# ramanathanlab/distllm

Hardware: NVIDIA B200
Metric: embedded chunks/sec @512-tok (higher is better)
Workload: dtype bf16

## Files before the change

### distllm_b200/_native.py

```python

from __future__ import annotations

import ctypes as C
from pathlib import Path

import torch

LIB_PATH = Path(__file__).resolve().parent / 'libb2e.so'
LIB_PATHS = {'f16': LIB_PATH, 'bf16': LIB_PATH.with_name('libb2e_bf16.so')}
STORAGE_TORCH_DTYPE = {'f16': torch.float16, 'bf16': torch.bfloat16}
_STORAGE_BY_ARCH = {'bert': 'bf16', 'esm': 'bf16', 'modernbert': 'bf16', 'mistral': 'f16'}


def storage_for_arch(arch: str) -> str:
    import os

    forced = os.environ.get('B2E_STORAGE')
    if forced:
        if forced not in LIB_PATHS:
            raise NativeError(f'B2E_STORAGE={forced!r}: expected one of {sorted(LIB_PATHS)}')
        return forced
    return _STORAGE_BY_ARCH[arch]


# ... 33 lines not shown
    'b2e_topk_ip',
    'b2e_topk_ip_tc',
    'b2e_max_row_norm',
    'b2e_pack_ubinary',
    'b2e_search_ubinary',
    'b2e_layernorm',
)
DEBUG_EXPORTS = (
    'b2e_debug_set_att3_clock',
    'b2e_debug_set_att3_flags',
    'b2e_debug_set_pair_flags',
    'b2e_debug_set_clock_buffer',
    'b2e_debug_set_layers',
    'b2e_debug_set_att3_variant',
    'b2e_debug_set_packing',
    'b2e_debug_topk_tc_fell_back',
    'b2e_debug_pack_layout',
    'b2e_debug_gemm_rows',
    'b2e_debug_attention_packed',
)


class NativeError(RuntimeError):
    """Raised when libb2e.so is missing or a native call fails."""


class ModelDesc(C.Structure):

    _fields_ = [
        ('arch', C.c_int32),
        ('num_layers', C.c_int32),
        ('hidden', C.c_int32),
        ('heads', C.c_int32),
# ... 249 lines not shown
                    epilogue: int, m_dev: torch.Tensor, out: torch.Tensor) -> torch.Tensor:
    lib = load(storage_of(a.dtype))
    for t, what in ((a, 'a'), (w, 'w'), (out, 'out'), (m_dev, 'm_dev')):
        _cuda_contig(t, what)
    if m_dev.dtype != torch.int32:
        raise NativeError('m_dev must be int32')
    m, k = a.shape
    n = w.shape[0]
    lib.b2e_debug_gemm_rows.argtypes = [C.c_void_p] * 5 + [C.c_int] * 4 + [C.c_void_p] * 2
    with torch.cuda.device(a.device):
        check(lib.b2e_debug_gemm_rows(a.data_ptr(), w.data_ptr(), _ptr(bias), _ptr(resid), out.data_ptr(), m, n, k,
                                      epilogue, m_dev.data_ptr(), stream_ptr(a.device)), lib)
    return out


def debug_attention_packed(qkv: torch.Tensor, attention_mask: torch.Tensor, cu: torch.Tensor, seq_len: torch.Tensor,
                           ctx: torch.Tensor, heads: int, kv_heads: int, head_dim: int, window: int = 0) -> torch.Tensor:
    lib = load(storage_of(qkv.dtype))
    for t, what in ((qkv, 'qkv'), (attention_mask, 'attention_mask'), (cu, 'cu'), (seq_len, 'len'), (ctx, 'ctx')):
        _cuda_contig(t, what)
    b, s = attention_mask.shape
    lib.b2e_debug_attention_packed.argtypes = [C.c_void_p] * 5 + [C.c_int] * 6 + [C.c_void_p]
    with torch.cuda.device(qkv.device):
        check(lib.b2e_debug_attention_packed(qkv.data_ptr(), attention_mask.data_ptr(), cu.data_ptr(),
                                             seq_len.data_ptr(), ctx.data_ptr(), b, s, heads, kv_heads, head_dim,
                                             window, stream_ptr(qkv.device)), lib)
    return ctx


def pack_ubinary(embeddings: torch.Tensor) -> torch.Tensor:
# ... 105 lines not shown
```

### distllm_b200/csrc/b2e_api.cu

```cuda
#include "../../include/b2e.h"
#include "../../include/b2e_debug.h"

#include <cuda.h>
#include <cuda_runtime.h>

#include <cstdarg>
#include <cstdio>
#include <cstdlib>
#include <cstring>
#include <string>
#include <utility>
#include <vector>

#include "attention3.cuh"
#include "attention4.cuh"
#include "attention5.cuh"
#include "binsearch.cuh"
#include "common.cuh"
#include "gemm.cuh"
#include "gemm2.cuh"
#include "mistral_ops.cuh"
#include "pack.cuh"
#include "rowops.cuh"
#include "topk.cuh"
// ... 217 lines not shown
bool g_gemm2_profiling = false;

template <int STAGES, int EPI>
int launch_gemm2_cfg(const CUtensorMap& ta, const CUtensorMap& tb, const CUtensorMap& tout,
                     const float* bias, const h16* resid, int M, int N, int K, int sms,
                     cudaStream_t st, const int* m_dev = nullptr) {
  using Cfg = Gemm2Cfg<STAGES>;
  const int tiles = ((M + 255) / 256) * (N / G2_BN);
  int grid = 2 * tiles;
  if (grid > (sms & ~1)) grid = sms & ~1;
  if constexpr (EPI == EPI_BIAS) {
    if (g_gemm2_profiling) {
      auto kern_tl = gemm2_h16_pair_kernel<STAGES, EPI, true>;
      const int arc = ensure_smem_attr(kern_tl, Cfg::SMEM_BYTES);
      if (arc) return arc;
      kern_tl<<<grid, G2_THREADS, Cfg::SMEM_BYTES, st>>>(ta, tb, tout, bias, resid, M, N, K, m_dev);
      CUDA_TRY(cudaGetLastError());
      return B2E_OK;
    }
  }
  auto kern = gemm2_h16_pair_kernel<STAGES, EPI>;
  {
    const int arc = ensure_smem_attr(kern, Cfg::SMEM_BYTES);
    if (arc) return arc;
  }
  kern<<<grid, G2_THREADS, Cfg::SMEM_BYTES, st>>>(ta, tb, tout, bias, resid, M, N, K, m_dev);
  CUDA_TRY(cudaGetLastError());
  return B2E_OK;
}

int launch_gemm(const CUtensorMap& ta, const CUtensorMap& tb, void* out, const float* bias,
                const void* resid, int M, int N, int K, int epi, int sms, cudaStream_t st,
                const int* m_dev = nullptr) {
  const h16* r = static_cast<const h16*>(resid);
  CUtensorMap tout;
  int rc;
  const bool glu = epi == B2E_EPI_SWIGLU || epi == B2E_EPI_GEGLU;
  const int n_out = glu ? N / 2 : N;
  if ((rc = make_tmap_h16(&tout, out, M, n_out, GEMM_OUT_BOX_ROWS))) return rc;
  if (N % 256 == 0 && gemm_use_pair()) {
    constexpr int PS = 5;
    switch (epi) {
      case B2E_EPI_BIAS: return launch_gemm2_cfg<PS, EPI_BIAS>(ta, tb, tout, bias, r, M, N, K, sms, st, m_dev);
      case B2E_EPI_BIAS_GELU: return launch_gemm2_cfg<PS, EPI_BIAS_GELU>(ta, tb, tout, bias, r, M, N, K, sms, st, m_dev);
      case B2E_EPI_BIAS_RESID: return launch_gemm2_cfg<PS, EPI_BIAS_RESID>(ta, tb, tout, bias, r, M, N, K, sms, st, m_dev);
      case B2E_EPI_SWIGLU: return launch_gemm2_cfg<PS, EPI_SWIGLU>(ta, tb, tout, bias, r, M, N, K, sms, st, m_dev);
      case B2E_EPI_GEGLU: return launch_gemm2_cfg<PS, EPI_GEGLU>(ta, tb, tout, bias, r, M, N, K, sms, st, m_dev);
    }
    return fail(B2E_ERR_INVALID, "unknown epilogue %d", epi);
  }
  if (N % 256 == 0) return launch_gemm_bn<256, 4>(ta, tb, tout, bias, r, M, N, K, epi, sms, st, m_dev);
  return launch_gemm_bn<128, 6>(ta, tb, tout, bias, r, M, N, K, epi, sms, st, m_dev);
}

struct AttnScratch {
  float* bias = nullptr;
  int* kv_chunks = nullptr;
  int* plain_chunks = nullptr;
  size_t cap_bias = 0, cap_b = 0;
  uint64_t gen = 0;
  int device = -1;
  int ensure(int B, int S_pad) {
    int dev = 0;
    CUDA_TRY(cudaGetDevice(&dev));
    if (dev != device) {
      release();
      device = dev;
// ... 389 lines not shown
    CUDA_TRY(cudaMalloc(&e->pk_src, sizeof(int) * tokens));
    e->pk_cap_t = tokens;
  }
  return e->pool.ensure(B, S, (size_t)B * pool_nsplit(S) * e->desc.hidden);
}

int g_packing = -1;
inline bool packing_enabled() {
  if (g_packing < 0) {
    const char* e = getenv("B2E_PACKED");
    g_packing = (e && e[0] == '0') ? 0 : 1;
  }
  return g_packing == 1;
}

int pack_prepare(B2EEncoder* e, const int64_t* mask, int B, int S, bool enable, cudaStream_t st, SeqLayout* lay) {
  pack_lengths_kernel<<<(B + 7) / 8, 256, 0, st>>>(mask, e->pk_len_raw, e->pk_ok, B, S);
  pack_scan_kernel<<<1, 256, 0, st>>>(e->pk_len_raw, e->pk_ok, e->pk_len, e->pk_cu, e->pk_treal, B, S,
                                      enable ? 1 : 0);
  pack_fill_kernel<<<dim3((S + 255) / 256, B), 256, 0, st>>>(e->pk_len, e->pk_cu, e->pk_src, B, S);
  CUDA_TRY(cudaGetLastError());
  lay->cu = e->pk_cu;
  lay->len = e->pk_len;
  lay->t_real = e->pk_treal;
  lay->tok_src = e->pk_src;
  return B2E_OK;
}

int validate_batch(const B2EEncoder* e, int B, int S) {
  if (!e) return fail(B2E_ERR_INVALID, "null encoder handle");
// ... 12 lines not shown
  const B2EModelDesc& d = e->desc;
  const int M = B * S, H = d.hidden, I = d.intermediate;
  int rc;
  DISPATCH_NV(H, (embed_layernorm_kernel<NV><<<row_blocks(M), ROW_THREADS, 0, st>>>(
                     ids, types, e->word(), e->pos(), e->type(), e->emb_g(), e->emb_b(), e->hidden,
                     M, S, d.eps, lay.t_real, lay.tok_src)));
  CUDA_TRY(cudaGetLastError());

  if ((rc = attention_prepare(e->attn, mask, B, S, st))) return rc;
  CUtensorMap tm_hidden, tm_ctx, tm_ffn, tm_qkv, tm_kv64;
  if ((rc = make_tmap_h16(&tm_kv64, e->qkv, M, 3 * H, AT3_KC))) return rc;
  if ((rc = make_tmap_h16(&tm_hidden, e->hidden, M, H, 128))) return rc;
  if ((rc = make_tmap_h16(&tm_ctx, e->ctx, M, H, 128))) return rc;
  if ((rc = make_tmap_h16(&tm_ffn, e->ffn, M, I, 128))) return rc;
  if ((rc = make_tmap_h16(&tm_qkv, e->qkv, M, 3 * H, 128))) return rc;

  for (int l = 0; l < d.num_layers; ++l) {
    if ((rc = launch_gemm(tm_hidden, e->tm_wqkv[l], e->qkv, (const float*)e->L(l, 1), nullptr, M,
                          3 * H, H, B2E_EPI_BIAS, e->sms, st, lay.t_real)))
      return rc;
    if ((rc = launch_attention(tm_qkv, tm_kv64, e->attn, e->ctx, B, S, d.heads, e->sms, st, 0, lay)))
      return rc;
    if ((rc = launch_gemm(tm_ctx, e->tm_wo[l], e->tmp, (const float*)e->L(l, 3), nullptr, M, H, H,
                          B2E_EPI_BIAS, e->sms, st, lay.t_real)))
      return rc;
    DISPATCH_NV(H, (layernorm_kernel<NV, h16><<<row_blocks(M), ROW_THREADS, 0, st>>>(
                       e->tmp, e->hidden, (const float*)e->L(l, 4), (const float*)e->L(l, 5),
                       e->hidden, M, d.eps, lay.t_real)));
    if ((rc = launch_gemm(tm_hidden, e->tm_w1[l], e->ffn, (const float*)e->L(l, 7), nullptr, M, I,
                          H, B2E_EPI_BIAS_GELU, e->sms, st, lay.t_real)))
      return rc;
    if ((rc = launch_gemm(tm_ffn, e->tm_w2[l], e->tmp, (const float*)e->L(l, 9), nullptr, M, H, I,
                          B2E_EPI_BIAS, e->sms, st, lay.t_real)))
      return rc;
    if (l + 1 < d.num_layers) {
      DISPATCH_NV(H, (layernorm_kernel<NV, h16><<<row_blocks(M), ROW_THREADS, 0, st>>>(
                         e->tmp, e->hidden, (const float*)e->L(l, 10), (const float*)e->L(l, 11),
                         e->hidden, M, d.eps, lay.t_real)));
    }
  }
  CUDA_TRY(cudaGetLastError());
  return B2E_OK;
}

int run_esm_trunk(B2EEncoder* e, const int64_t* ids, const int64_t* mask, int B, int S,
                  cudaStream_t st, const SeqLayout& lay = SeqLayout()) {
  const B2EModelDesc& d = e->desc;
  const int M = B * S, H = d.hidden, I = d.intermediate, L = d.num_layers;
  const int mask_token = d.reserved - 1;
  int rc;
  esm_token_scale_kernel<<<(B + 7) / 8, 256, 0, st>>>(ids, mask, e->tok_scale, B, S, mask_token);
  DISPATCH_NV(H, (esm_embed_kernel<NV><<<row_blocks(M), ROW_THREADS, 0, st>>>(
                     ids, mask, (const float*)e->w[0], e->tok_scale, e->xres, M, S, mask_token, lay.t_real,
// ... 145 lines not shown
int b2e_storage_dtype(void) { return kStorageDtype; }

int b2e_debug_set_att3_clock(void* device_buffer) {
  long long* p = static_cast<long long*>(device_buffer);
  CUDA_TRY(cudaMemcpyToSymbol(g_att3_clock, &p, sizeof(p)));
  return B2E_OK;
}

int b2e_debug_set_att3_flags(int flags) {
  CUDA_TRY(cudaMemcpyToSymbol(g_att3_flags, &flags, sizeof(flags)));
  return B2E_OK;
}

int b2e_debug_set_packing(int on) {
  g_packing = on ? 1 : 0;
  return B2E_OK;
}

int b2e_debug_set_att3_variant(int variant) {
  g_att3_variant = variant;
  return B2E_OK;
}

int b2e_debug_set_pair_flags(int flags) {
  g_gemm2_profiling = flags != 0;
  CUDA_TRY(cudaMemcpyToSymbol(g_gemm2_flags, &flags, sizeof(flags)));
  return B2E_OK;
}

int b2e_debug_set_clock_buffer(void* device_buffer) {
// ... 563 lines not shown
  if ((rc = make_tmap_h16(&tb, W, N, K, gemm_bn_for(N)))) return rc;
  return launch_gemm(ta, tb, out, bias, resid, M, N, K, epi, info.sms, (cudaStream_t)stream, m_dev);
}

int b2e_gemm_h16(const void* A, const void* W, const float* bias, const void* resid, void* out,
                  int M, int N, int K, int epi, void* stream) {
  return gemm_h16_checked(A, W, bias, resid, out, M, N, K, epi, nullptr, stream);
}

int b2e_debug_gemm_rows(const void* A, const void* W, const float* bias, const void* resid, void* out,
                        int M, int N, int K, int epi, const int* m_dev, void* stream) {
  if (!m_dev) return fail(B2E_ERR_INVALID, "gemm_rows: null device row count");
  return gemm_h16_checked(A, W, bias, resid, out, M, N, K, epi, m_dev, stream);
}

int b2e_attention_d64(const void* qkv, const int64_t* mask, void* ctx, int B, int S, int heads,
                      float* dbg, void* stream) {
  if (!qkv || !mask || !ctx) return fail(B2E_ERR_INVALID, "null tensor pointer");
  if (B <= 0 || S <= 0 || heads <= 0) return fail(B2E_ERR_INVALID, "empty attention problem");
  if (dbg) return fail(B2E_ERR_UNSUPPORTED, "the score dump of the first attention kernel is gone: pass NULL");
  int rc;
  DeviceInfo info;
  if ((rc = current_device_info(&info))) return rc;
  cudaStream_t st = (cudaStream_t)stream;
  CUtensorMap tq, tkv;
  if ((rc = make_tmap_h16(&tq, qkv, (uint64_t)B * S, (uint64_t)3 * heads * AT3_D, 128))) return rc;
  if ((rc = make_tmap_h16(&tkv, qkv, (uint64_t)B * S, (uint64_t)3 * heads * AT3_D, AT3_KC))) return rc;
  if ((rc = attention_prepare(g_attn_scratch, mask, B, S, st))) return rc;
  return launch_attention(tq, tkv, g_attn_scratch, ctx, B, S, heads, info.sms, st);
}
// ... 417 lines not shown
```

### distllm_b200/csrc/common.cuh

```cuda
#pragma once

#include <cuda.h>
#include <cuda_bf16.h>
#include <cuda_fp16.h>
#include <cuda_runtime.h>
#include <stdint.h>

namespace b2e {

using bf16 = __nv_bfloat16;
#ifdef B2E_STORAGE_BF16
using h16 = __nv_bfloat16;
#else
using h16 = __half;
#endif

__device__ __forceinline__ uint32_t smem_u32(const void* p) {
  return static_cast<uint32_t>(__cvta_generic_to_shared(p));
}

__device__ __forceinline__ uint32_t lane_id() { return threadIdx.x & 31u; }

__device__ __forceinline__ bool elect_one() {
  uint32_t pred = 0;
// ... 223 lines not shown
}
__device__ __forceinline__ void mbar_wait_cluster(uint32_t bar, uint32_t parity) {
  uint32_t ok = 0;
  while (!ok) {
    asm volatile(
        "{\n\t"
        ".reg .pred p;\n\t"
        "mbarrier.try_wait.parity.acquire.cluster.shared::cta.b64 p, [%1], %2;\n\t"
        "selp.u32 %0, 1, 0, p;\n\t"
        "}\n"
        : "=r"(ok)
        : "r"(bar), "r"(parity)
        : "memory");
  }
}
__device__ __forceinline__ void tma_load_2d_pair(uint32_t dst, const CUtensorMap* m,
                                                 uint32_t bar_cluster_addr, int c0, int c1) {
  asm volatile(
      "cp.async.bulk.tensor.2d.cta_group::2.shared::cluster.global.mbarrier::complete_tx::bytes"
      " [%0], [%1, {%3, %4}], [%2];"
      ::"r"(dst), "l"(m), "r"(bar_cluster_addr), "r"(c0), "r"(c1)
      : "memory");
}
__device__ __forceinline__ void tmem_alloc_pair(uint32_t smem_dst, uint32_t ncols) {
  asm volatile("tcgen05.alloc.cta_group::2.sync.aligned.shared::cta.b32 [%0], %1;" ::"r"(smem_dst),
               "r"(ncols)
               : "memory");
  asm volatile("tcgen05.relinquish_alloc_permit.cta_group::2.sync.aligned;" ::: "memory");
}
__device__ __forceinline__ void tmem_dealloc_pair(uint32_t taddr, uint32_t ncols) {
// ... 125 lines not shown
```

### distllm_b200/csrc/gemm.cuh

```cuda
#pragma once

#include "common.cuh"

namespace b2e {

enum GemmEpi : int { EPI_BIAS = 0, EPI_BIAS_GELU = 1, EPI_BIAS_RESID = 2, EPI_SWIGLU = 3, EPI_GEGLU = 4 };
__host__ __device__ constexpr bool epi_is_glu(int epi) { return epi == EPI_SWIGLU || epi == EPI_GEGLU; }

constexpr int GEMM_BM = 128;
constexpr int GEMM_BK = 64;
constexpr int GEMM_THREADS = 384;
constexpr int GEMM_EPI_WARPS = 8;
constexpr int GEMM_OUT_BOX_ROWS = 32;
constexpr int GEMM_STAGING_BYTES = GEMM_OUT_BOX_ROWS * 128;

template <int BN, int STAGES>
struct GemmCfg {
  static constexpr int A_BYTES = GEMM_BM * GEMM_BK * 2;
  static constexpr int B_BYTES = BN * GEMM_BK * 2;
  static constexpr int STAGE_BYTES = A_BYTES + B_BYTES;
  static constexpr int STAGING_OFFSET = STAGES * STAGE_BYTES;
  static constexpr int BAR_OFFSET = STAGING_OFFSET + GEMM_EPI_WARPS * GEMM_STAGING_BYTES;
  static constexpr int BIAS_OFFSET = BAR_OFFSET + 256;
  static constexpr int SMEM_BYTES = BIAS_OFFSET + 2 * BN * 4;
// ... 326 lines not shown
```

### distllm_b200/csrc/gemm2.cuh

```cuda
#pragma once

#include "common.cuh"
#include "gemm.cuh"

namespace b2e {

constexpr int G2_BN = 256;
constexpr int G2_THREADS = 384;
constexpr int G2_EPI_WARPS = 8;

template <int STAGES>
struct Gemm2Cfg {
  static constexpr int A_BYTES = 128 * GEMM_BK * 2;
  static constexpr int B_BYTES = (G2_BN / 2) * GEMM_BK * 2;
  static constexpr int STAGE_BYTES = A_BYTES + B_BYTES;
  static constexpr int STAGING_OFFSET = STAGES * STAGE_BYTES;
  static constexpr int STAGING_PER_WARP = 2 * GEMM_STAGING_BYTES;
  static constexpr int BAR_OFFSET = STAGING_OFFSET + G2_EPI_WARPS * STAGING_PER_WARP;
  static constexpr int SMEM_BYTES = BAR_OFFSET + 256;
  static constexpr int TMEM_COLS = 2 * G2_BN;
  static_assert(SMEM_BYTES <= 232448, "exceeds the 227 KiB per-CTA shared memory limit");
};

__device__ long long* g_gemm2_clock = nullptr;
__device__ int g_gemm2_flags = 0;

template <int STAGES, int EPI, bool TL = false>
__global__ void __cluster_dims__(2, 1, 1) __launch_bounds__(G2_THREADS, 1)
gemm2_h16_pair_kernel(const __grid_constant__ CUtensorMap tm_a,
                       const __grid_constant__ CUtensorMap tm_b,
                       const __grid_constant__ CUtensorMap tm_out,
                       const float* __restrict__ bias, const h16* __restrict__ resid, int M, int N,
                       int K, const int* __restrict__ m_dev) {
  if (m_dev != nullptr) M = __ldg(m_dev);
  using Cfg = Gemm2Cfg<STAGES>;
  extern __shared__ __align__(1024) uint8_t smem[];
  const uint32_t smem_base = smem_u32(smem);
  if ((smem_base & 1023u) != 0) __trap();

  const uint32_t full_bar = smem_base + Cfg::BAR_OFFSET;
  const uint32_t empty_bar = full_bar + 8u * STAGES;
  const uint32_t tfull_bar = empty_bar + 8u * STAGES;
  const uint32_t tempty_bar = tfull_bar + 16u;
  volatile uint32_t* tmem_slot =
      reinterpret_cast<volatile uint32_t*>(smem + Cfg::BAR_OFFSET + 8 * (2 * STAGES + 4));

  const int warp = threadIdx.x >> 5;
  const int lane = threadIdx.x & 31;
  const int flags = TL ? g_gemm2_flags : 0;
  const uint32_t rank = cluster_ctarank();
  const bool leader = rank == 0;

  if (warp == 0 && elect_one()) {
    tma_prefetch_desc(&tm_a);
    tma_prefetch_desc(&tm_b);
    tma_prefetch_desc(&tm_out);
  }
  if (warp == 1 && elect_one()) {
    for (int s = 0; s < STAGES; ++s) {
      mbar_init(full_bar + 8u * s, 1);
      mbar_init(empty_bar + 8u * s, 1);
    }
    for (int s = 0; s < 2; ++s) {
      mbar_init(tfull_bar + 8u * s, 1);
      mbar_init(tempty_bar + 8u * s, 2 * G2_EPI_WARPS);
    }
    mbar_fence_init();
  }
  cluster_sync_all();
  if (warp == 2) tmem_alloc_pair(smem_u32(const_cast<uint32_t*>(tmem_slot)), Cfg::TMEM_COLS);
  tc_fence_before();
  __syncthreads();
  tc_fence_after();
  const uint32_t tmem_base = *tmem_slot;

  const int m_pairs = (M + 255) / 256;
  const int n_tiles = N / G2_BN;
  const int total = m_pairs * n_tiles;
  const int kblocks = K / GEMM_BK;
  const int cluster_id = blockIdx.x >> 1;
  const int n_clusters = gridDim.x >> 1;
  long long* const clk = (TL && blockIdx.x < 2) ? g_gemm2_clock : nullptr;
  int clk_n = 0;
#define G2_STAMP(role)                                                                       \
  do {                                                                                       \
    if constexpr (TL) {                                                                      \
      if (clk != nullptr && clk_n < 256) clk[(blockIdx.x * 2 + (role)) * 256 + clk_n++] = clock64(); \
    }                                                                                        \
  } while (0)

  if (warp == 0) {
    if (elect_one()) {
      const uint32_t lead_full0 = mapa_shared(full_bar, 0);
      int stage = 0;
      uint32_t phase = 0;
      for (int tile = cluster_id; tile < total; tile += n_clusters) {
        const int m_pair = tile / n_tiles, n_blk = tile % n_tiles;
        const int row_a = m_pair * 256 + static_cast<int>(rank) * 128;
        const int row_b = n_blk * G2_BN + static_cast<int>(rank) * (G2_BN / 2);
        for (int kb = 0; kb < kblocks; ++kb) {
          mbar_wait(empty_bar + 8u * stage, phase ^ 1u);
          G2_STAMP(0);
          const uint32_t a_dst = smem_base + stage * Cfg::STAGE_BYTES;
          if (flags & 4) {
            if (leader) mbar_arrive(full_bar + 8u * stage);
          } else {
            if (leader) mbar_expect_tx(full_bar + 8u * stage, 2 * Cfg::STAGE_BYTES);
            const uint32_t fb = lead_full0 + 8u * stage;
            tma_load_2d_pair(a_dst, &tm_a, fb, kb * GEMM_BK, row_a);
            tma_load_2d_pair(a_dst + Cfg::A_BYTES, &tm_b, fb, kb * GEMM_BK, row_b);
          }
          if (++stage == STAGES) { stage = 0; phase ^= 1u; }
        }
      }
    }
  } else if (warp == 1) {
    if (leader && elect_one()) {
      constexpr uint32_t idesc = make_idesc_h16(256, G2_BN, 0, 0);
      int stage = 0;
      uint32_t phase = 0;
      int local = 0;
      for (int tile = cluster_id; tile < total; tile += n_clusters, ++local) {
        const int as = local & 1;
        const uint32_t aphase = (local >> 1) & 1u;
        mbar_wait_cluster(tempty_bar + 8u * as, aphase ^ 1u);
        tc_fence_after();
        const uint32_t d_tmem = tmem_base + static_cast<uint32_t>(as * G2_BN);
        for (int kb = 0; kb < kblocks; ++kb) {
          G2_STAMP(1);
          mbar_wait(full_bar + 8u * stage, phase);
          G2_STAMP(1);
          tc_fence_after();
          const uint32_t a_addr = smem_base + stage * Cfg::STAGE_BYTES;
          const uint64_t a_desc = make_smem_desc_sw128(a_addr, 16, 1024);
          const uint64_t b_desc = make_smem_desc_sw128(a_addr + Cfg::A_BYTES, 16, 1024);
          if (!(flags & 2)) {
#pragma unroll
            for (int k = 0; k < GEMM_BK / 16; ++k)
              tc_mma_f16_ss_pair(d_tmem, a_desc + 2u * k, b_desc + 2u * k, idesc,
                                 static_cast<uint32_t>((kb | k) != 0));
          }
          tc_commit_pair(empty_bar + 8u * stage, 3);
          G2_STAMP(1);
          if (++stage == STAGES) { stage = 0; phase ^= 1u; }
        }
        tc_commit_pair(tfull_bar + 8u * as, 3);
      }
    }
  } else if (warp >= 4) {
    const int q = warp & 3;
    const int half = (warp - 4) >> 2;
    constexpr int COLS_PER_WARP = G2_BN / 2;
    uint8_t* staging = smem + Cfg::STAGING_OFFSET + (warp - 4) * Cfg::STAGING_PER_WARP;
    const uint32_t staging_addr = smem_base + Cfg::STAGING_OFFSET + (warp - 4) * Cfg::STAGING_PER_WARP;
    const uint32_t lead_tempty0 = mapa_shared(tempty_bar, 0);
    const bool stamp = (warp == 4 && lane == 0 && !leader);
    int local = 0;
    for (int tile = cluster_id; tile < total; tile += n_clusters, ++local) {
      const int m_pair = tile / n_tiles, n_blk = tile % n_tiles;
      const int as = local & 1;
      const uint32_t aphase = (local >> 1) & 1u;
      const int row0 = m_pair * 256 + static_cast<int>(rank) * 128 + q * 32;
      const int row = row0 + lane;
      const bool row_ok = row < M;
      const int col0 = half * COLS_PER_WARP;
      const int gcol0 = n_blk * G2_BN + col0;
      const h16* resid_row =
          (EPI == EPI_BIAS_RESID) ? resid + static_cast<size_t>(row) * N + gcol0 : nullptr;

      if (stamp) G2_STAMP(1);
      if (flags & 16) {
        while (!mbar_test(tfull_bar + 8u * as, aphase)) __nanosleep(256);
      } else {
        mbar_wait(tfull_bar + 8u * as, aphase);
      }
      if (stamp) G2_STAMP(1);
      tc_fence_after();
      const uint32_t t_base = tmem_base + (static_cast<uint32_t>(q * 32) << 16) +
                              static_cast<uint32_t>(as * G2_BN + col0);
      if constexpr (epi_is_glu(EPI)) {
        uint32_t g[2][32], u[2][32];
        tmem_ld32(t_base, g[0]);
        tmem_ld32(t_base + 32u, g[1]);
        tmem_ld32(t_base + 64u, u[0]);
        tmem_ld32(t_base + 96u, u[1]);
        if (lane == 0) tma_store_wait_read<1>();
        __syncwarp();
        tmem_ld_wait();
        if (!(flags & 1)) {
          const int sidx = local & 1;
          gemm_swiglu_chunk<EPI == EPI_GEGLU>(g, u, staging + sidx * GEMM_STAGING_BYTES, lane);
          fence_proxy_async_smem();
          __syncwarp();
          if (lane == 0 && row0 < M) {
// ... 45 lines not shown
```

### include/b2e_debug.h

```cpp
#ifndef B2E_DEBUG_H_
#define B2E_DEBUG_H_

#include <stdint.h>

#ifdef __cplusplus
extern "C" {
#endif

struct B2EEncoder;
int b2e_debug_set_layers(struct B2EEncoder* enc, int n_layers);

int b2e_debug_set_att3_clock(void* device_buffer);
int b2e_debug_set_att3_flags(int flags);
int b2e_debug_set_packing(int on);
int b2e_debug_topk_tc_fell_back(int* out);
int b2e_debug_set_att3_variant(int variant);
int b2e_debug_set_pair_flags(int flags);
int b2e_debug_set_clock_buffer(void* device_buffer);

int b2e_debug_pack_layout(const int64_t* mask, int B, int S, int enable, int* cu, int* len, int* t_real,
                          int* tok_src, void* stream);
int b2e_debug_gemm_rows(const void* A, const void* W, const float* bias, const void* resid, void* out, int M,
                        int N, int K, int epi, const int* m_dev, void* stream);
int b2e_debug_attention_packed(const void* qkv, const int64_t* mask, const int* cu, const int* len, void* ctx,
                               int B, int S, int heads, int kv_heads, int head_dim, int window, void* stream);

#ifdef __cplusplus
}
#endif
#endif
```

Measured before the change: 9767.

## Fuse residual add and LayerNorm into the CTA-pair GEMM epilogue via cluster row-stat exchange

Adds a LayerNorm epilogue to the 2-CTA tcgen05 GEMM for BERT's attention-output and FFN-down projections. Clusters of 2*NP CTAs now cover the full hidden row (N<=1024). Each CTA TMA-loads the residual tile, computes partial mean and variance from TMEM, and exchanges them across the cluster with st.async. This removes the separate layernorm kernel launches and the round trip of the tmp buffer through global memory. In exchange, large clusters cap how many run at once and the grid is limited to M/256 clusters, which may underuse the SMs.

```diff
diff --git a/distllm_b200/_native.py b/distllm_b200/_native.py
--- a/distllm_b200/_native.py
+++ b/distllm_b200/_native.py
@@ -71,9 +71,12 @@
     'b2e_debug_set_layers',
     'b2e_debug_set_att3_variant',
     'b2e_debug_set_packing',
+    'b2e_debug_set_ln_fusion',
     'b2e_debug_topk_tc_fell_back',
     'b2e_debug_pack_layout',
     'b2e_debug_gemm_rows',
+    'b2e_debug_gemm_ln',
+    'b2e_debug_gemm_ln_max_clusters',
     'b2e_debug_attention_packed',
 )
 
@@ -353,6 +356,40 @@
     return out
 
 
+def debug_set_ln_fusion(on: bool, storage: str = 'bf16') -> None:
+    lib = load(storage)
+    lib.b2e_debug_set_ln_fusion.argtypes = [C.c_int]
+    check(lib.b2e_debug_set_ln_fusion(int(bool(on))), lib)
+
+
+def debug_gemm_ln(a: torch.Tensor, w: torch.Tensor, bias: torch.Tensor | None, resid: torch.Tensor,
+                  gamma: torch.Tensor, beta: torch.Tensor, eps: float, out: torch.Tensor,
+                  m_dev: torch.Tensor | None = None) -> torch.Tensor:
+    lib = load(storage_of(a.dtype))
+    for t, what in ((a, 'a'), (w, 'w'), (resid, 'resid'), (gamma, 'gamma'), (beta, 'beta'), (out, 'out')):
+        _cuda_contig(t, what)
+    if gamma.dtype != torch.float32 or beta.dtype != torch.float32:
+        raise NativeError('gamma and beta must be float32')
+    if m_dev is not None and m_dev.dtype != torch.int32:
+        raise NativeError('m_dev must be int32')
+    m, k = a.shape
+    n = w.shape[0]
+    lib.b2e_debug_gemm_ln.argtypes = [C.c_void_p] * 6 + [C.c_float, C.c_void_p] + [C.c_int] * 3 + [C.c_void_p] * 2
+    with torch.cuda.device(a.device):
+        check(lib.b2e_debug_gemm_ln(a.data_ptr(), w.data_ptr(), _ptr(bias), resid.data_ptr(), gamma.data_ptr(),
+                                    beta.data_ptr(), float(eps), out.data_ptr(), m, n, k, _ptr(m_dev),
+                                    stream_ptr(a.device)), lib)
+    return out
+
+
+def debug_gemm_ln_max_clusters(n: int, storage: str = 'bf16') -> int:
+    lib = load(storage)
+    out = C.c_int(0)
+    lib.b2e_debug_gemm_ln_max_clusters.argtypes = [C.c_int, C.POINTER(C.c_int)]
+    check(lib.b2e_debug_gemm_ln_max_clusters(n, C.byref(out)), lib)
+    return int(out.value)
+
+
 def debug_attention_packed(qkv: torch.Tensor, attention_mask: torch.Tensor, cu: torch.Tensor, seq_len: torch.Tensor,
                            ctx: torch.Tensor, heads: int, kv_heads: int, head_dim: int, window: int = 0) -> torch.Tensor:
     lib = load(storage_of(qkv.dtype))
diff --git a/distllm_b200/csrc/b2e_api.cu b/distllm_b200/csrc/b2e_api.cu
--- a/distllm_b200/csrc/b2e_api.cu
+++ b/distllm_b200/csrc/b2e_api.cu
@@ -255,7 +255,7 @@
       auto kern_tl = gemm2_h16_pair_kernel<STAGES, EPI, true>;
       const int arc = ensure_smem_attr(kern_tl, Cfg::SMEM_BYTES);
       if (arc) return arc;
-      kern_tl<<<grid, G2_THREADS, Cfg::SMEM_BYTES, st>>>(ta, tb, tout, bias, resid, M, N, K, m_dev);
+      kern_tl<<<grid, G2_THREADS, Cfg::SMEM_BYTES, st>>>(ta, tb, tout, tout, bias, resid, M, N, K, m_dev, G2Ln());
       CUDA_TRY(cudaGetLastError());
       return B2E_OK;
     }
@@ -265,7 +265,7 @@
     const int arc = ensure_smem_attr(kern, Cfg::SMEM_BYTES);
     if (arc) return arc;
   }
-  kern<<<grid, G2_THREADS, Cfg::SMEM_BYTES, st>>>(ta, tb, tout, bias, resid, M, N, K, m_dev);
+  kern<<<grid, G2_THREADS, Cfg::SMEM_BYTES, st>>>(ta, tb, tout, tout, bias, resid, M, N, K, m_dev, G2Ln());
   CUDA_TRY(cudaGetLastError());
   return B2E_OK;
 }
@@ -292,6 +292,77 @@
   }
   if (N % 256 == 0) return launch_gemm_bn<256, 4>(ta, tb, tout, bias, r, M, N, K, epi, sms, st, m_dev);
   return launch_gemm_bn<128, 6>(ta, tb, tout, bias, r, M, N, K, epi, sms, st, m_dev);
+}
+
+template <typename Kern>
+int max_active_clusters(Kern kern, int cluster, int smem_bytes, int* out) {
+  static std::vector<std::pair<std::pair<const void*, int>, int>> done;
+  int dev = 0;
+  CUDA_TRY(cudaGetDevice(&dev));
+  const void* key = reinterpret_cast<const void*>(kern);
+  for (const auto& d : done)
+    if (d.first.first == key && d.first.second == dev) {
+      *out = d.second;
+      return B2E_OK;
+    }
+  cudaLaunchConfig_t cfg = {};
+  cfg.gridDim = dim3(cluster);
+  cfg.blockDim = dim3(G2_THREADS);
+  cfg.dynamicSmemBytes = smem_bytes;
+  int n = 0;
+  CUDA_TRY(cudaOccupancyMaxActiveClusters(&n, kern, &cfg));
+  if (n <= 0) return fail(B2E_ERR_CUDA, "no cluster of %d CTAs with %d B of shared memory fits the device", cluster, smem_bytes);
+  done.push_back({{key, dev}, n});
+  *out = n;
+  return B2E_OK;
+}
+
+inline bool gemm_ln_eligible(int N) { return gemm_use_pair() && N % 256 == 0 && N / 256 <= 4; }
+
+constexpr int LN_STAGES = 4;
+
+template <int NP>
+int launch_gemm_ln_np(const CUtensorMap& ta, const CUtensorMap& tb, const CUtensorMap& tout,
+                      const CUtensorMap& tres, const float* bias, const G2Ln& ln, int M, int N, int K,
+                      cudaStream_t st, const int* m_dev) {
+  using Cfg = Gemm2Cfg<LN_STAGES, NP>;
+  auto kern = gemm2_h16_pair_kernel<LN_STAGES, EPI_BIAS_RESID_LN, false, NP>;
+  int rc;
+  if ((rc = ensure_smem_attr(kern, Cfg::SMEM_BYTES))) return rc;
+  int clusters = 0;
+  if ((rc = max_active_clusters(kern, 2 * NP, Cfg::SMEM_BYTES, &clusters))) return rc;
+  const int m_pairs = (M + 255) / 256;
+  if (clusters > m_pairs) clusters = m_pairs;
+  cudaLaunchConfig_t cfg = {};
+  cfg.gridDim = dim3(2 * NP * clusters);
+  cfg.blockDim = dim3(G2_THREADS);
+  cfg.dynamicSmemBytes = Cfg::SMEM_BYTES;
+  cfg.stream = st;
+  CUDA_TRY(cudaLaunchKernelEx(&cfg, kern, ta, tb, tout, tres, bias, static_cast<const h16*>(nullptr), M, N, K,
+                              m_dev, ln));
+  return B2E_OK;
+}
+
+int launch_gemm_ln(const CUtensorMap& ta, const CUtensorMap& tb, void* out, const void* resid, const float* bias,
+                   const float* gamma, const float* beta, float eps, int M, int N, int K, cudaStream_t st,
+                   const int* m_dev = nullptr) {
+  if (!gemm_ln_eligible(N)) return fail(B2E_ERR_INVALID, "gemm + LayerNorm: N=%d needs N %% 256 == 0, N <= 1024 and the CTA-pair GEMM", N);
+  CUtensorMap tout, tres;
+  int rc;
+  if ((rc = make_tmap_h16(&tout, out, M, N, GEMM_OUT_BOX_ROWS))) return rc;
+  if (resid == out) tres = tout;
+  else if ((rc = make_tmap_h16(&tres, resid, M, N, GEMM_OUT_BOX_ROWS))) return rc;
+  G2Ln ln;
+  ln.gamma = gamma;
+  ln.beta = beta;
+  ln.eps = eps;
+  switch (N / 256) {
+    case 1: return launch_gemm_ln_np<1>(ta, tb, tout, tres, bias, ln, M, N, K, st, m_dev);
+    case 2: return launch_gemm_ln_np<2>(ta, tb, tout, tres, bias, ln, M, N, K, st, m_dev);
+    case 3: return launch_gemm_ln_np<3>(ta, tb, tout, tres, bias, ln, M, N, K, st, m_dev);
+    case 4: return launch_gemm_ln_np<4>(ta, tb, tout, tres, bias, ln, M, N, K, st, m_dev);
+  }
+  return fail(B2E_ERR_INVALID, "gemm + LayerNorm: N=%d", N);
 }
 
 struct AttnScratch {
@@ -711,6 +782,15 @@
   return g_packing == 1;
 }
 
+int g_ln_fusion = -1;
+inline bool ln_fusion_enabled() {
+  if (g_ln_fusion < 0) {
+    const char* e = getenv("B2E_LN_FUSE");
+    g_ln_fusion = (e && e[0] == '0') ? 0 : 1;
+  }
+  return g_ln_fusion == 1;
+}
+
 int pack_prepare(B2EEncoder* e, const int64_t* mask, int B, int S, bool enable, cudaStream_t st, SeqLayout* lay) {
   pack_lengths_kernel<<<(B + 7) / 8, 256, 0, st>>>(mask, e->pk_len_raw, e->pk_ok, B, S);
   pack_scan_kernel<<<1, 256, 0, st>>>(e->pk_len_raw, e->pk_ok, e->pk_len, e->pk_cu, e->pk_treal, B, S,
@@ -753,6 +833,7 @@
   if ((rc = make_tmap_h16(&tm_ctx, e->ctx, M, H, 128))) return rc;
   if ((rc = make_tmap_h16(&tm_ffn, e->ffn, M, I, 128))) return rc;
   if ((rc = make_tmap_h16(&tm_qkv, e->qkv, M, 3 * H, 128))) return rc;
+  const bool fuse_ln = ln_fusion_enabled() && gemm_ln_eligible(H);
 
   for (int l = 0; l < d.num_layers; ++l) {
     if ((rc = launch_gemm(tm_hidden, e->tm_wqkv[l], e->qkv, (const float*)e->L(l, 1), nullptr, M,
@@ -760,22 +841,37 @@
       return rc;
     if ((rc = launch_attention(tm_qkv, tm_kv64, e->attn, e->ctx, B, S, d.heads, e->sms, st, 0, lay)))
       return rc;
-    if ((rc = launch_gemm(tm_ctx, e->tm_wo[l], e->tmp, (const float*)e->L(l, 3), nullptr, M, H, H,
-                          B2E_EPI_BIAS, e->sms, st, lay.t_real)))
-      return rc;
-    DISPATCH_NV(H, (layernorm_kernel<NV, h16><<<row_blocks(M), ROW_THREADS, 0, st>>>(
-                       e->tmp, e->hidden, (const float*)e->L(l, 4), (const float*)e->L(l, 5),
-                       e->hidden, M, d.eps, lay.t_real)));
+    if (fuse_ln) {
+      if ((rc = launch_gemm_ln(tm_ctx, e->tm_wo[l], e->hidden, e->hidden, (const float*)e->L(l, 3),
+                               (const float*)e->L(l, 4), (const float*)e->L(l, 5), d.eps, M, H, H, st,
+                               lay.t_real)))
+        return rc;
+    } else {
+      if ((rc = launch_gemm(tm_ctx, e->tm_wo[l], e->tmp, (const float*)e->L(l, 3), nullptr, M, H, H,
+                            B2E_EPI_BIAS, e->sms, st, lay.t_real)))
+        return rc;
+      DISPATCH_NV(H, (layernorm_kernel<NV, h16><<<row_blocks(M), ROW_THREADS, 0, st>>>(
+                         e->tmp, e->hidden, (const float*)e->L(l, 4), (const float*)e->L(l, 5),
+                         e->hidden, M, d.eps, lay.t_real)));
+    }
     if ((rc = launch_gemm(tm_hidden, e->tm_w1[l], e->ffn, (const float*)e->L(l, 7), nullptr, M, I,
                           H, B2E_EPI_BIAS_GELU, e->sms, st, lay.t_real)))
       return rc;
-    if ((rc = launch_gemm(tm_ffn, e->tm_w2[l], e->tmp, (const float*)e->L(l, 9), nullptr, M, H, I,
-                          B2E_EPI_BIAS, e->sms, st, lay.t_real)))
-      return rc;
-    if (l + 1 < d.num_layers) {
-      DISPATCH_NV(H, (layernorm_kernel<NV, h16><<<row_blocks(M), ROW_THREADS, 0, st>>>(
-                         e->tmp, e->hidden, (const float*)e->L(l, 10), (const float*)e->L(l, 11),
-                         e->hidden, M, d.eps, lay.t_real)));
+    const bool last = l + 1 == d.num_layers;
+    if (fuse_ln && !last) {
+      if ((rc = launch_gemm_ln(tm_ffn, e->tm_w2[l], e->hidden, e->hidden, (const float*)e->L(l, 9),
+                               (const float*)e->L(l, 10), (const float*)e->L(l, 11), d.eps, M, H, I, st,
+                               lay.t_real)))
+        return rc;
+    } else {
+      if ((rc = launch_gemm(tm_ffn, e->tm_w2[l], e->tmp, (const float*)e->L(l, 9), nullptr, M, H, I,
+                            B2E_EPI_BIAS, e->sms, st, lay.t_real)))
+        return rc;
+      if (!last) {
+        DISPATCH_NV(H, (layernorm_kernel<NV, h16><<<row_blocks(M), ROW_THREADS, 0, st>>>(
+                           e->tmp, e->hidden, (const float*)e->L(l, 10), (const float*)e->L(l, 11),
+                           e->hidden, M, d.eps, lay.t_real)));
+      }
     }
   }
   CUDA_TRY(cudaGetLastError());
@@ -951,6 +1047,11 @@
 
 int b2e_debug_set_packing(int on) {
   g_packing = on ? 1 : 0;
+  return B2E_OK;
+}
+
+int b2e_debug_set_ln_fusion(int on) {
+  g_ln_fusion = on ? 1 : 0;
   return B2E_OK;
 }
 
@@ -1544,6 +1645,43 @@
   return gemm_h16_checked(A, W, bias, resid, out, M, N, K, epi, m_dev, stream);
 }
 
+int b2e_debug_gemm_ln(const void* A, const void* W, const float* bias, const void* resid, const float* gamma,
+                      const float* beta, float eps, void* out, int M, int N, int K, const int* m_dev,
+                      void* stream) {
+  if (!A || !W || !resid || !gamma || !beta || !out) return fail(B2E_ERR_INVALID, "null tensor pointer");
+  int rc;
+  if ((rc = check_gemm_shape(M, N, K))) return rc;
+  DeviceInfo info;
+  if ((rc = current_device_info(&info))) return rc;
+  CUtensorMap ta, tb;
+  if ((rc = make_tmap_h16(&ta, A, M, K, 128))) return rc;
+  if ((rc = make_tmap_h16(&tb, W, N, K, gemm_bn_for(N)))) return rc;
+  return launch_gemm_ln(ta, tb, out, resid, bias, gamma, beta, eps, M, N, K, (cudaStream_t)stream, m_dev);
+}
+
+int b2e_debug_gemm_ln_max_clusters(int N, int* clusters) {
+  if (!clusters) return fail(B2E_ERR_INVALID, "null output pointer");
+  if (!gemm_ln_eligible(N)) return fail(B2E_ERR_INVALID, "gemm + LayerNorm: N=%d is not eligible", N);
+  int rc;
+  DeviceInfo info;
+  if ((rc = current_device_info(&info))) return rc;
+  switch (N / 256) {
+#define B2E_LN_CLUSTERS(NP)                                                                                \
+  case NP: {                                                                                               \
+    auto kern = gemm2_h16_pair_kernel<LN_STAGES, EPI_BIAS_RESID_LN, false, NP>;                            \
+    using Cfg = Gemm2Cfg<LN_STAGES, NP>;                                                                   \
+    if ((rc = ensure_smem_attr(kern, Cfg::SMEM_BYTES))) return rc;                                         \
+    return max_active_clusters(kern, 2 * NP, Cfg::SMEM_BYTES, clusters);                                   \
+  }
+    B2E_LN_CLUSTERS(1)
+    B2E_LN_CLUSTERS(2)
+    B2E_LN_CLUSTERS(3)
+    B2E_LN_CLUSTERS(4)
+#undef B2E_LN_CLUSTERS
+  }
+  return fail(B2E_ERR_INVALID, "gemm + LayerNorm: N=%d", N);
+}
+
 int b2e_attention_d64(const void* qkv, const int64_t* mask, void* ctx, int B, int S, int heads,
                       float* dbg, void* stream) {
   if (!qkv || !mask || !ctx) return fail(B2E_ERR_INVALID, "null tensor pointer");
diff --git a/distllm_b200/csrc/common.cuh b/distllm_b200/csrc/common.cuh
--- a/distllm_b200/csrc/common.cuh
+++ b/distllm_b200/csrc/common.cuh
@@ -261,6 +261,11 @@
         : "memory");
   }
 }
+__device__ __forceinline__ void st_async_f32x2(uint32_t cluster_addr, float a, float b, uint32_t bar_cluster_addr) {
+  asm volatile("st.async.shared::cluster.mbarrier::complete_tx::bytes.v2.f32 [%0], {%1, %2}, [%3];"
+               ::"r"(cluster_addr), "f"(a), "f"(b), "r"(bar_cluster_addr)
+               : "memory");
+}
 __device__ __forceinline__ void tma_load_2d_pair(uint32_t dst, const CUtensorMap* m,
                                                  uint32_t bar_cluster_addr, int c0, int c1) {
   asm volatile(
diff --git a/distllm_b200/csrc/gemm.cuh b/distllm_b200/csrc/gemm.cuh
--- a/distllm_b200/csrc/gemm.cuh
+++ b/distllm_b200/csrc/gemm.cuh
@@ -4,7 +4,9 @@
 
 namespace b2e {
 
-enum GemmEpi : int { EPI_BIAS = 0, EPI_BIAS_GELU = 1, EPI_BIAS_RESID = 2, EPI_SWIGLU = 3, EPI_GEGLU = 4 };
+enum GemmEpi : int {
+  EPI_BIAS = 0, EPI_BIAS_GELU = 1, EPI_BIAS_RESID = 2, EPI_SWIGLU = 3, EPI_GEGLU = 4, EPI_BIAS_RESID_LN = 5
+};
 __host__ __device__ constexpr bool epi_is_glu(int epi) { return epi == EPI_SWIGLU || epi == EPI_GEGLU; }
 
 constexpr int GEMM_BM = 128;
diff --git a/distllm_b200/csrc/gemm2.cuh b/distllm_b200/csrc/gemm2.cuh
--- a/distllm_b200/csrc/gemm2.cuh
+++ b/distllm_b200/csrc/gemm2.cuh
@@ -9,7 +9,7 @@
 constexpr int G2_THREADS = 384;
 constexpr int G2_EPI_WARPS = 8;
 
-template <int STAGES>
+template <int STAGES, int XCHG_NP = 0>
 struct Gemm2Cfg {
   static constexpr int A_BYTES = 128 * GEMM_BK * 2;
   static constexpr int B_BYTES = (G2_BN / 2) * GEMM_BK * 2;
@@ -17,23 +17,37 @@
   static constexpr int STAGING_OFFSET = STAGES * STAGE_BYTES;
   static constexpr int STAGING_PER_WARP = 2 * GEMM_STAGING_BYTES;
   static constexpr int BAR_OFFSET = STAGING_OFFSET + G2_EPI_WARPS * STAGING_PER_WARP;
-  static constexpr int SMEM_BYTES = BAR_OFFSET + 256;
+  static constexpr int RES_BAR_OFFSET = BAR_OFFSET + 128;
+  static constexpr int XCHG_BAR_OFFSET = BAR_OFFSET + 192;
+  static constexpr int XCHG_OFFSET = BAR_OFFSET + 256;
+  static constexpr int XCHG_BYTES = 2 * XCHG_NP * 2 * 128 * 8;
+  static constexpr int SMEM_BYTES = XCHG_OFFSET + XCHG_BYTES;
   static constexpr int TMEM_COLS = 2 * G2_BN;
+  static_assert(8 * (2 * STAGES + 4) + 4 <= 128, "ring barriers overlap the LayerNorm barriers");
   static_assert(SMEM_BYTES <= 232448, "exceeds the 227 KiB per-CTA shared memory limit");
 };
 
+struct G2Ln {
+  const float* gamma = nullptr;
+  const float* beta = nullptr;
+  float eps = 0.0f;
+};
+
 __device__ long long* g_gemm2_clock = nullptr;
 __device__ int g_gemm2_flags = 0;
 
-template <int STAGES, int EPI, bool TL = false>
-__global__ void __cluster_dims__(2, 1, 1) __launch_bounds__(G2_THREADS, 1)
+template <int STAGES, int EPI, bool TL = false, int NP = 1>
+__global__ void __cluster_dims__(2 * NP, 1, 1) __launch_bounds__(G2_THREADS, 1)
 gemm2_h16_pair_kernel(const __grid_constant__ CUtensorMap tm_a,
                        const __grid_constant__ CUtensorMap tm_b,
                        const __grid_constant__ CUtensorMap tm_out,
+                       const __grid_constant__ CUtensorMap tm_res,
                        const float* __restrict__ bias, const h16* __restrict__ resid, int M, int N,
-                       int K, const int* __restrict__ m_dev) {
+                       int K, const int* __restrict__ m_dev, const G2Ln ln) {
   if (m_dev != nullptr) M = __ldg(m_dev);
-  using Cfg = Gemm2Cfg<STAGES>;
+  constexpr bool LN = EPI == EPI_BIAS_RESID_LN;
+  static_assert(!LN || !TL, "the LayerNorm epilogue has no profiling instantiation");
+  using Cfg = Gemm2Cfg<STAGES, LN ? NP : 0>;
   extern __shared__ __align__(1024) uint8_t smem[];
   const uint32_t smem_base = smem_u32(smem);
   if ((smem_base & 1023u) != 0) __trap();
@@ -42,6 +56,8 @@
   const uint32_t empty_bar = full_bar + 8u * STAGES;
   const uint32_t tfull_bar = empty_bar + 8u * STAGES;
   const uint32_t tempty_bar = tfull_bar + 16u;
+  const uint32_t res_bar0 = smem_base + Cfg::RES_BAR_OFFSET;
+  const uint32_t xchg_bar0 = smem_base + Cfg::XCHG_BAR_OFFSET;
   volatile uint32_t* tmem_slot =
       reinterpret_cast<volatile uint32_t*>(smem + Cfg::BAR_OFFSET + 8 * (2 * STAGES + 4));
 
@@ -49,12 +65,17 @@
   const int lane = threadIdx.x & 31;
   const int flags = TL ? g_gemm2_flags : 0;
   const uint32_t rank = cluster_ctarank();
-  const bool leader = rank == 0;
+  const uint32_t lead = rank & ~1u;
+  const uint32_t prank = rank & 1u;
+  const bool leader = prank == 0;
+  const int pair = static_cast<int>(rank >> 1);
+  const uint16_t pair_mask = static_cast<uint16_t>(3u << lead);
 
   if (warp == 0 && elect_one()) {
     tma_prefetch_desc(&tm_a);
     tma_prefetch_desc(&tm_b);
     tma_prefetch_desc(&tm_out);
+    if constexpr (LN) tma_prefetch_desc(&tm_res);
   }
   if (warp == 1 && elect_one()) {
     for (int s = 0; s < STAGES; ++s) {
@@ -64,6 +85,10 @@
     for (int s = 0; s < 2; ++s) {
       mbar_init(tfull_bar + 8u * s, 1);
       mbar_init(tempty_bar + 8u * s, 2 * G2_EPI_WARPS);
+    }
+    if constexpr (LN) {
+      for (int w = 0; w < G2_EPI_WARPS; ++w) mbar_init(res_bar0 + 8u * w, 1);
+      for (int b = 0; b < 8; ++b) mbar_init(xchg_bar0 + 8u * b, 1);
     }
     mbar_fence_init();
   }
@@ -78,8 +103,10 @@
   const int n_tiles = N / G2_BN;
   const int total = m_pairs * n_tiles;
   const int kblocks = K / GEMM_BK;
-  const int cluster_id = blockIdx.x >> 1;
-  const int n_clusters = gridDim.x >> 1;
+  const int cluster_id = blockIdx.x / (2 * NP);
+  const int n_clusters = gridDim.x / (2 * NP);
+  const int tile0 = NP > 1 || LN ? cluster_id * n_tiles + pair : cluster_id;
+  const int tile_step = NP > 1 || LN ? n_clusters * n_tiles : n_clusters;
   long long* const clk = (TL && blockIdx.x < 2) ? g_gemm2_clock : nullptr;
   int clk_n = 0;
 #define G2_STAMP(role)                                                                       \
@@ -91,13 +118,13 @@
 
   if (warp == 0) {
     if (elect_one()) {
-      const uint32_t lead_full0 = mapa_shared(full_bar, 0);
+      const uint32_t lead_full0 = mapa_shared(full_bar, lead);
       int stage = 0;
       uint32_t phase = 0;
-      for (int tile = cluster_id; tile < total; tile += n_clusters) {
+      for (int tile = tile0; tile < total; tile += tile_step) {
         const int m_pair = tile / n_tiles, n_blk = tile % n_tiles;
-        const int row_a = m_pair * 256 + static_cast<int>(rank) * 128;
-        const int row_b = n_blk * G2_BN + static_cast<int>(rank) * (G2_BN / 2);
+        const int row_a = m_pair * 256 + static_cast<int>(prank) * 128;
+        const int row_b = n_blk * G2_BN + static_cast<int>(prank) * (G2_BN / 2);
         for (int kb = 0; kb < kblocks; ++kb) {
           mbar_wait(empty_bar + 8u * stage, phase ^ 1u);
           G2_STAMP(0);
@@ -120,7 +147,7 @@
       int stage = 0;
       uint32_t phase = 0;
       int local = 0;
-      for (int tile = cluster_id; tile < total; tile += n_clusters, ++local) {
+      for (int tile = tile0; tile < total; tile += tile_step, ++local) {
         const int as = local & 1;
         const uint32_t aphase = (local >> 1) & 1u;
         mbar_wait_cluster(tempty_bar + 8u * as, aphase ^ 1u);
@@ -140,11 +167,11 @@
               tc_mma_f16_ss_pair(d_tmem, a_desc + 2u * k, b_desc + 2u * k, idesc,
                                  static_cast<uint32_t>((kb | k) != 0));
           }
-          tc_commit_pair(empty_bar + 8u * stage, 3);
+          tc_commit_pair(empty_bar + 8u * stage, pair_mask);
           G2_STAMP(1);
           if (++stage == STAGES) { stage = 0; phase ^= 1u; }
         }
-        tc_commit_pair(tfull_bar + 8u * as, 3);
+        tc_commit_pair(tfull_bar + 8u * as, pair_mask);
       }
     }
   } else if (warp >= 4) {
@@ -153,20 +180,30 @@
     constexpr int COLS_PER_WARP = G2_BN / 2;
     uint8_t* staging = smem + Cfg::STAGING_OFFSET + (warp - 4) * Cfg::STAGING_PER_WARP;
     const uint32_t staging_addr = smem_base + Cfg::STAGING_OFFSET + (warp - 4) * Cfg::STAGING_PER_WARP;
-    const uint32_t lead_tempty0 = mapa_shared(tempty_bar, 0);
+    const uint32_t lead_tempty0 = mapa_shared(tempty_bar, lead);
     const bool stamp = (warp == 4 && lane == 0 && !leader);
     int local = 0;
-    for (int tile = cluster_id; tile < total; tile += n_clusters, ++local) {
+    for (int tile = tile0; tile < total; tile += tile_step, ++local) {
       const int m_pair = tile / n_tiles, n_blk = tile % n_tiles;
       const int as = local & 1;
       const uint32_t aphase = (local >> 1) & 1u;
-      const int row0 = m_pair * 256 + static_cast<int>(rank) * 128 + q * 32;
+      const int row0 = m_pair * 256 + static_cast<int>(prank) * 128 + q * 32;
       const int row = row0 + lane;
       const bool row_ok = row < M;
       const int col0 = half * COLS_PER_WARP;
       const int gcol0 = n_blk * G2_BN + col0;
       const h16* resid_row =
           (EPI == EPI_BIAS_RESID) ? resid + static_cast<size_t>(row) * N + gcol0 : nullptr;
+      const uint32_t res_bar = res_bar0 + 8u * static_cast<uint32_t>(warp - 4);
+
+      if constexpr (LN) {
+        if (lane == 0) {
+          tma_store_wait_read<0>();
+          mbar_expect_tx(res_bar, 2 * GEMM_STAGING_BYTES);
+          tma_load_2d(staging_addr, &tm_res, res_bar, gcol0, row0);
+          tma_load_2d(staging_addr + GEMM_STAGING_BYTES, &tm_res, res_bar, gcol0 + 64, row0);
+        }
+      }
 
       if (stamp) G2_STAMP(1);
       if (flags & 16) {
@@ -178,6 +215,128 @@
       tc_fence_after();
       const uint32_t t_base = tmem_base + (static_cast<uint32_t>(q * 32) << 16) +
                               static_cast<uint32_t>(as * G2_BN + col0);
+      if constexpr (LN) {
+        mbar_wait(res_bar, static_cast<uint32_t>(local & 1));
+        float sp[4] = {0.f, 0.f, 0.f, 0.f};
+#pragma unroll 1
+        for (int c = 0; c < COLS_PER_WARP / 32; ++c) {
+          uint32_t acc[32];
+          tmem_ld32(t_base + static_cast<uint32_t>(c * 32), acc);
+          tmem_ld_wait();
+          const uint8_t* st_tile = staging + (c >> 1) * GEMM_STAGING_BYTES + lane * 128;
+#pragma unroll
+          for (int u4 = 0; u4 < 4; ++u4) {
+            const int u = (c & 1) * 4 + u4;
+            float4 b0 = make_float4(0.f, 0.f, 0.f, 0.f), b1 = b0;
+            if (bias != nullptr) {
+              b0 = __ldg(reinterpret_cast<const float4*>(bias + gcol0 + c * 32 + u4 * 8));
+              b1 = __ldg(reinterpret_cast<const float4*>(bias + gcol0 + c * 32 + u4 * 8 + 4));
+            }
+            uint32_t* a = &acc[u4 * 8];
+            const float2 y0 = unpack_h16x2(pack_h16x2(__uint_as_float(a[0]) + b0.x, __uint_as_float(a[1]) + b0.y));
+            const float2 y1 = unpack_h16x2(pack_h16x2(__uint_as_float(a[2]) + b0.z, __uint_as_float(a[3]) + b0.w));
+            const float2 y2 = unpack_h16x2(pack_h16x2(__uint_as_float(a[4]) + b1.x, __uint_as_float(a[5]) + b1.y));
+            const float2 y3 = unpack_h16x2(pack_h16x2(__uint_as_float(a[6]) + b1.z, __uint_as_float(a[7]) + b1.w));
+            const uint4 rr = *reinterpret_cast<const uint4*>(st_tile + ((u ^ (lane & 7)) << 4));
+            const float2 r0 = unpack_h16x2(rr.x), r1 = unpack_h16x2(rr.y), r2 = unpack_h16x2(rr.z),
+                         r3 = unpack_h16x2(rr.w);
+            const float x[8] = {y0.x + r0.x, y0.y + r0.y, y1.x + r1.x, y1.y + r1.y,
+                                y2.x + r2.x, y2.y + r2.y, y3.x + r3.x, y3.y + r3.y};
+#pragma unroll
+            for (int e = 0; e < 8; ++e) {
+              sp[e & 3] += x[e];
+              a[e] = __float_as_uint(x[e]);
+            }
+          }
+          tmem_st32(t_base + static_cast<uint32_t>(c * 32), acc);
+        }
+        tmem_st_wait();
+        const float mean_s = ((sp[0] + sp[1]) + (sp[2] + sp[3])) * (1.0f / COLS_PER_WARP);
+        float qp[4] = {0.f, 0.f, 0.f, 0.f};
+#pragma unroll 1
+        for (int c = 0; c < COLS_PER_WARP / 64; ++c) {
+          uint32_t v[2][32];
+          tmem_ld32(t_base + static_cast<uint32_t>(c * 64), v[0]);
+          tmem_ld32(t_base + static_cast<uint32_t>(c * 64 + 32), v[1]);
+          tmem_ld_wait();
+#pragma unroll
+          for (int i = 0; i < 64; ++i) {
+            const float d = __uint_as_float(v[i >> 5][i & 31]) - mean_s;
+            qp[i & 3] = fmaf(d, d, qp[i & 3]);
+          }
+        }
+        const float2 part = make_float2(mean_s, (qp[0] + qp[1]) + (qp[2] + qp[3]));
+
+        const int buf = local & 1;
+        const uint32_t xbar = xchg_bar0 + 8u * static_cast<uint32_t>(buf * 4 + q);
+        if (half == 0 && lane == 0) mbar_expect_tx(xbar, 2 * NP * 32 * 8);
+        const uint32_t slot = smem_base + Cfg::XCHG_OFFSET +
+                              static_cast<uint32_t>((((buf * NP + pair) * 2 + half) * 128 + q * 32 + lane) * 8);
+#pragma unroll
+        for (int p = 0; p < NP; ++p) {
+          const uint32_t dst = static_cast<uint32_t>(2 * p) + prank;
+          st_async_f32x2(mapa_shared(slot, dst), part.x, part.y, mapa_shared(xbar, dst));
+        }
+        mbar_wait_cluster(xbar, static_cast<uint32_t>((local >> 1) & 1));
+        const float2* xs = reinterpret_cast<const float2*>(smem + Cfg::XCHG_OFFSET) + buf * NP * 2 * 128 + q * 32 + lane;
+        float2 pt[2 * NP];
+        float msum = 0.0f;
+#pragma unroll
+        for (int i = 0; i < 2 * NP; ++i) {
+          pt[i] = xs[i * 128];
+          msum += pt[i].x;
+        }
+        const float mean = msum / static_cast<float>(2 * NP);
+        float m2 = 0.0f;
+#pragma unroll
+        for (int i = 0; i < 2 * NP; ++i) {
+          const float d = pt[i].x - mean;
+          m2 += fmaf(128.0f * d, d, pt[i].y);
+        }
+        const float rstd = rsqrtf(m2 * (1.0f / (NP * G2_BN)) + ln.eps);
+
+#pragma unroll 1
+        for (int c = 0; c < COLS_PER_WARP / 64; ++c) {
+          uint32_t v[2][32];
+          tmem_ld32(t_base + static_cast<uint32_t>(c * 64), v[0]);
+          tmem_ld32(t_base + static_cast<uint32_t>(c * 64 + 32), v[1]);
+          tmem_ld_wait();
+#pragma unroll
+          for (int u = 0; u < 8; ++u) {
+            const int col = gcol0 + c * 64 + u * 8;
+            const float4 g0 = __ldg(reinterpret_cast<const float4*>(ln.gamma + col));
+            const float4 g1 = __ldg(reinterpret_cast<const float4*>(ln.gamma + col + 4));
+            const float4 e0 = __ldg(reinterpret_cast<const float4*>(ln.beta + col));
+            const float4 e1 = __ldg(reinterpret_cast<const float4*>(ln.beta + col + 4));
+            const uint32_t* xi = &v[u >> 2][(u & 3) * 8];
+            const float g[8] = {g0.x, g0.y, g0.z, g0.w, g1.x, g1.y, g1.z, g1.w};
+            const float e[8] = {e0.x, e0.y, e0.z, e0.w, e1.x, e1.y, e1.z, e1.w};
+            float y[8];
+#pragma unroll
+            for (int k = 0; k < 8; ++k) y[k] = fmaf((__uint_as_float(xi[k]) - mean) * rstd, g[k], e[k]);
+            uint4 o;
+            o.x = pack_h16x2(y[0], y[1]);
+            o.y = pack_h16x2(y[2], y[3]);
+            o.z = pack_h16x2(y[4], y[5]);
+            o.w = pack_h16x2(y[6], y[7]);
+            *reinterpret_cast<uint4*>(staging + c * GEMM_STAGING_BYTES + lane * 128 + ((u ^ (lane & 7)) << 4)) = o;
+          }
+        }
+        tc_fence_before();
+        __syncwarp();
+        if (lane == 0) {
+          if (leader) mbar_arrive(tempty_bar + 8u * as);
+          else mbar_arrive_cluster_relaxed(lead_tempty0 + 8u * as);
+        }
+        fence_proxy_async_smem();
+        __syncwarp();
+        if (lane == 0 && row0 < M) {
+          tma_store_2d(&tm_out, staging_addr, gcol0, row0);
+          tma_store_2d(&tm_out, staging_addr + GEMM_STAGING_BYTES, gcol0 + 64, row0);
+          tma_store_commit();
+        }
+        continue;
+      }
       if constexpr (epi_is_glu(EPI)) {
         uint32_t g[2][32], u[2][32];
         tmem_ld32(t_base, g[0]);
diff --git a/include/b2e_debug.h b/include/b2e_debug.h
--- a/include/b2e_debug.h
+++ b/include/b2e_debug.h
@@ -14,6 +14,7 @@
 int b2e_debug_set_att3_flags(int flags);
 int b2e_debug_set_packing(int on);
 int b2e_debug_topk_tc_fell_back(int* out);
+int b2e_debug_set_ln_fusion(int on);
 int b2e_debug_set_att3_variant(int variant);
 int b2e_debug_set_pair_flags(int flags);
 int b2e_debug_set_clock_buffer(void* device_buffer);
@@ -22,6 +23,9 @@
                           int* tok_src, void* stream);
 int b2e_debug_gemm_rows(const void* A, const void* W, const float* bias, const void* resid, void* out, int M,
                         int N, int K, int epi, const int* m_dev, void* stream);
+int b2e_debug_gemm_ln(const void* A, const void* W, const float* bias, const void* resid, const float* gamma,
+                      const float* beta, float eps, void* out, int M, int N, int K, const int* m_dev, void* stream);
+int b2e_debug_gemm_ln_max_clusters(int N, int* clusters);
 int b2e_debug_attention_packed(const void* qkv, const int64_t* mask, const int* cu, const int* len, void* ctx,
                                int B, int S, int heads, int kv_heads, int head_dim, int window, void* stream);
 
```

After: 10180 (median of 6 runs). 1.04x the previous value.
